# zacz08/ADM

Hardware: AMD Instinct MI355X
Metric: train images/sec (CIFAR-10 32x32 uncond DDM UNet, 1 optimizer step/iter) + 10-step sample images/sec (higher is better)
Workload: dtype f32; 1 GPU; BASELINE configs[1]: CIFAR-10 32x32 uncond two-decoder DhariwalUNet (216M params), bs=128/GPU fp32, ddm_const schedule, dropout 0.1, loss_simple (LPIPS term needs unfetchable VGG16 weights), clip 1.0 + AdamW + EMA(every 8); global_batch=128, image=3x32x32, parallelism=dp1, valid=True

## Files before the change

### adm_amd/csrc/conv_gemm_x6.hip

```cpp
#include "common.h"
#include "split_format.h"
#include <type_traits>

namespace {

struct G6P {
  const float* x; const unsigned short* w; const float* bias; const float* res; float* y;
  int M, N, K, ldx, ldy, ldr, wrows, tilesN, xbytes, wbytes, ybytes, rbytes;
  const float* amax_x; float wscale;
  float* amax_y;
};

typedef __attribute__((address_space(3))) void g6_lds_void;
constexpr int GM = 128, GN = 128, GCH = 2;
template <int FMT> struct G6Fmt {
  static constexpr int TERMS = split_terms(FMT);
  static constexpr int IMG = GCH * TERMS * 128 * 16;
  static constexpr int QW = 2 * TERMS;
};
constexpr int G_RA = 2, G_RB = 4, G_D = 4;

template <int FMT>
__global__ __launch_bounds__(512) void gemm_x6_kernel(G6P p) {
  constexpr int G_IMG = G6Fmt<FMT>::IMG, TERMS = G6Fmt<FMT>::TERMS, QW = G6Fmt<FMT>::QW;
  float sa = 1.f, inv_scale = 1.f;
  if (FMT) { sa = split_scale(adm_amax_read(p.amax_x)); inv_scale = 1.f / (sa * p.wscale); }
  extern __shared__ __attribute__((aligned(16))) unsigned short smg[];
  unsigned short* As = smg;
  unsigned short* Bs = smg + G_RA * G_IMG;
  const int tid = threadIdx.x, lane = tid & 63, hw_wid = tid >> 6;
  const bool producer = hw_wid >= 4;
  const int wid = hw_wid & 3;
  const int bid = adm_xcd_remap(blockIdx.x, gridDim.x);
  const int tilesM = gridDim.x / p.tilesN;
  const int tm = bid % tilesM, tn = bid / tilesM;
  const int m0 = tm * GM, n0 = tn * GN;
  const int S = p.K >> 5;
  constexpr unsigned OOB = 0x80000000u;

  if (producer) {
    const __amdgpu_buffer_rsrc_t rs_x = __builtin_amdgcn_make_buffer_rsrc(const_cast<float*>(p.x), 0, p.xbytes, 0x00020000);
    const int ptid = wid * 64 + lane;
    const int prow = ptid >> 3, quad = ptid & 7;
    unsigned voff[4];
#pragma unroll
    for (int j = 0; j < 4; ++j) {
      const int m = m0 + prow + 32 * j;
      voff[j] = (m < p.M) ? (unsigned)(((long)m * p.ldx + quad * 4) * 4) : OOB;
    }
    const int aq = quad & 3, ch = quad >> 2;
    unsigned short* la[4];
#pragma unroll
    for (int j = 0; j < 4; ++j) {
      const int row = prow + 32 * j;
      la[j] = As + (ch * TERMS * 128 + row) * 16 + ((((aq >> 1) ^ (row >> 3)) & 1) << 3) + (aq & 1) * 4;
    }
    f32x4 d[G_D][4];
    auto issue = [&](int set, int s) {
      const int soff = s << 7;
#pragma unroll
      for (int j = 0; j < 4; ++j)
        d[set][j] = __builtin_bit_cast(f32x4, __builtin_amdgcn_raw_buffer_load_b128(rs_x, (int)(s < S ? voff[j] : OOB), soff, 0));
    };
    auto store = [&](int set, int slot) {
#pragma unroll
      for (int j = 0; j < 4; ++j) {
        unsigned short* l = la[j] + slot * G_IMG;
        if (FMT) {
          u32x2 h0, h1;
          split2_quad(d[set][j], sa, h0, h1);
          *reinterpret_cast<u32x2*>(l) = h0;
          *reinterpret_cast<u32x2*>(l + 128 * 16) = h1;
          continue;
        }
        u32x2 t0, t1, t2;
        split3_quad(d[set][j], t0, t1, t2);
        *reinterpret_cast<u32x2*>(l) = t0;
        *reinterpret_cast<u32x2*>(l + 128 * 16) = t1;
        *reinterpret_cast<u32x2*>(l + 2 * 128 * 16) = t2;
      }
    };
#pragma unroll
    for (int k = 0; k < G_D; ++k) issue(k, k);
    __builtin_amdgcn_sched_barrier(0);
    for (int s0 = 0; s0 < S; s0 += G_D) {
#pragma unroll
      for (int k = 0; k < G_D; ++k) {
        if (s0 + k < S) {
          store(k, k & 1);
          __builtin_amdgcn_sched_barrier(0);
          issue(k, s0 + k + G_D);
          __builtin_amdgcn_sched_barrier(0);
          adm_lds_barrier();
        }
      }
    }
    return;
  }

  const __amdgpu_buffer_rsrc_t rs_w = __builtin_amdgcn_make_buffer_rsrc(const_cast<unsigned short*>(p.w), 0, p.wbytes, 0x00020000);
  const int wm = wid >> 1, wn = wid & 1;
  const int lr = lane & 31, lh = lane >> 5;
  unsigned b_voff[QW];
#pragma unroll
  for (int i = 0; i < QW; ++i) {
    const int q = wid * QW + i, img = q >> 2;
    const int row = (q & 3) * 32 + (lane >> 1);
    const int n = n0 + row;
    const int half = (lane ^ (row >> 3)) & 1;
    b_voff[i] = (n < p.wrows) ? (unsigned)((((long)img * p.wrows + n) * 16 + half * 8) * 2) : OOB;
  }
  int ld_s = 0, ld_slot = 0;
  auto issue_b = [&]() {
    const int kb = (ld_s * GCH * TERMS * p.wrows) << 5;
    unsigned short* dst = Bs + ld_slot * G_IMG + (wid * QW) * 512;
#pragma unroll
    for (int i = 0; i < QW; ++i)
      __builtin_amdgcn_raw_ptr_buffer_load_lds(rs_w, (g6_lds_void*)(dst + i * 512), 16, (int)b_voff[i], kb, 0, 0);
    ++ld_s;
    if (++ld_slot == G_RB) ld_slot = 0;
  };

  f32x16 acc[2][2], tot[2][2];
#pragma unroll
  for (int a = 0; a < 2; ++a)
#pragma unroll
    for (int b = 0; b < 2; ++b)
#pragma unroll
      for (int r = 0; r < 16; ++r) tot[a][b][r] = 0.f;
  const int fh = ((lh ^ (lr >> 3)) & 1) * 8;
  const int a_foff = (wm * 64 + lr) * 16 + fh;
  const int b_foff = (wn * 64 + lr) * 16 + fh;
  const f32x16 zero = {0.f, 0.f, 0.f, 0.f, 0.f, 0.f, 0.f, 0.f, 0.f, 0.f, 0.f, 0.f, 0.f, 0.f, 0.f, 0.f};

  issue_b();
  if (S > 1) issue_b();
  if (S > 2) issue_b();
  int slot_b = 0;
  for (int s = 0; s < S; ++s) {
    if (s + 2 < S) { if (FMT) asm volatile("s_waitcnt vmcnt(8) lgkmcnt(0)\n\ts_barrier" ::: "memory"); else asm volatile("s_waitcnt vmcnt(12) lgkmcnt(0)\n\ts_barrier" ::: "memory"); }
    else if (s + 1 < S) { if (FMT) asm volatile("s_waitcnt vmcnt(4) lgkmcnt(0)\n\ts_barrier" ::: "memory"); else asm volatile("s_waitcnt vmcnt(6) lgkmcnt(0)\n\ts_barrier" ::: "memory"); }
    else asm volatile("s_waitcnt vmcnt(0) lgkmcnt(0)\n\ts_barrier" ::: "memory");
    if (s + 3 < S) issue_b();
    const unsigned short* Ab = As + (s & 1) * G_IMG + a_foff;
    const unsigned short* Bb = Bs + slot_b * G_IMG + b_foff;
    if (++slot_b == G_RB) slot_b = 0;
    const bool first = (s & 1) == 0;
#pragma unroll
    for (int ch = 0; ch < GCH; ++ch) {
      bf16x8 a[2][TERMS], b[2][TERMS];
#pragma unroll
      for (int k = 0; k < TERMS; ++k)
#pragma unroll
        for (int blk = 0; blk < 2; ++blk) {
          a[blk][k] = __builtin_bit_cast(bf16x8, *reinterpret_cast<const u32x4*>(Ab + ((ch * TERMS + k) * 128 + blk * 32) * 16));
          b[blk][k] = __builtin_bit_cast(bf16x8, *reinterpret_cast<const u32x4*>(Bb + ((ch * TERMS + k) * 128 + blk * 32) * 16));
        }
#pragma unroll
      for (int mi = 0; mi < 2; ++mi)
#pragma unroll
        for (int ni = 0; ni < 2; ++ni) {
          f32x16 c;
          if (FMT) {
            const f16x8 a0 = __builtin_bit_cast(f16x8, a[mi][0]), a1 = __builtin_bit_cast(f16x8, a[mi][1]);
            const f16x8 b0 = __builtin_bit_cast(f16x8, b[ni][0]), b1 = __builtin_bit_cast(f16x8, b[ni][1]);
            c = __builtin_amdgcn_mfma_f32_32x32x16_f16(a0, b1, (first && ch == 0) ? zero : acc[mi][ni], 0, 0, 0);
            c = __builtin_amdgcn_mfma_f32_32x32x16_f16(a1, b0, c, 0, 0, 0);
            acc[mi][ni] = __builtin_amdgcn_mfma_f32_32x32x16_f16(a0, b0, c, 0, 0, 0);
            continue;
          }
          if (first && ch == 0) c = __builtin_amdgcn_mfma_f32_32x32x16_bf16(a[mi][0], b[ni][TERMS - 1], zero, 0, 0, 0);
          else c = __builtin_amdgcn_mfma_f32_32x32x16_bf16(a[mi][0], b[ni][TERMS - 1], acc[mi][ni], 0, 0, 0);
#ifndef G6_HALF
          c = __builtin_amdgcn_mfma_f32_32x32x16_bf16(a[mi][TERMS - 1], b[ni][0], c, 0, 0, 0);
          c = __builtin_amdgcn_mfma_f32_32x32x16_bf16(a[mi][1], b[ni][1], c, 0, 0, 0);
          c = __builtin_amdgcn_mfma_f32_32x32x16_bf16(a[mi][0], b[ni][1], c, 0, 0, 0);
#endif
          c = __builtin_amdgcn_mfma_f32_32x32x16_bf16(a[mi][1], b[ni][0], c, 0, 0, 0);
          acc[mi][ni] = __builtin_amdgcn_mfma_f32_32x32x16_bf16(a[mi][0], b[ni][0], c, 0, 0, 0);
        }
    }
    if (!first || s + 1 == S) {
#pragma unroll
      for (int mi = 0; mi < 2; ++mi)
#pragma unroll
        for (int ni = 0; ni < 2; ++ni) tot[mi][ni] += acc[mi][ni];
    }
  }

  const __amdgpu_buffer_rsrc_t rs_y = __builtin_amdgcn_make_buffer_rsrc(p.y, 0, p.ybytes, 0x00020000);
  const __amdgpu_buffer_rsrc_t rs_r = __builtin_amdgcn_make_buffer_rsrc(const_cast<float*>(p.res), 0, p.res ? p.rbytes : 0, 0x00020000);
  float am = 0.f;
  auto epilogue = [&](auto res_tag) {
    constexpr bool RES = decltype(res_tag)::value;
    float bv[2];
#pragma unroll
    for (int ni = 0; ni < 2; ++ni) {
      const int n = n0 + wn * 64 + ni * 32 + lr;
      bv[ni] = (p.bias && n < p.N) ? p.bias[n] : 0.f;
    }
    float v[2][2][16];
    unsigned n4[2], cmask[2], oy[2][16];
#pragma unroll
    for (int ni = 0; ni < 2; ++ni) {
      const int n = n0 + wn * 64 + ni * 32 + lr;
      n4[ni] = (unsigned)n * 4u;
      cmask[ni] = n < p.N ? 0u : OOB;
    }
    if (RES) {
      unsigned orr[2][16];
#pragma unroll
      for (int mi = 0; mi < 2; ++mi)
#pragma unroll
        for (int r = 0; r < 16; ++r) {
          const int m = m0 + wm * 64 + mi * 32 + 4 * lh + (r & 3) + 8 * (r >> 2);
          orr[mi][r] = m < p.M ? (unsigned)m * (unsigned)p.ldr * 4u : OOB;
        }
#pragma unroll
      for (int ni = 0; ni < 2; ++ni)
#pragma unroll
        for (int mi = 0; mi < 2; ++mi)
#pragma unroll
          for (int r = 0; r < 16; ++r)
            v[ni][mi][r] = __builtin_bit_cast(float, __builtin_amdgcn_raw_buffer_load_b32(rs_r, (int)max(orr[mi][r] + n4[ni], cmask[ni]), 0, 0));
      __builtin_amdgcn_sched_barrier(0);
    }
#pragma unroll
    for (int mi = 0; mi < 2; ++mi)
#pragma unroll
      for (int r = 0; r < 16; ++r) {
        const int m = m0 + wm * 64 + mi * 32 + 4 * lh + (r & 3) + 8 * (r >> 2);
        oy[mi][r] = m < p.M ? (unsigned)m * (unsigned)p.ldy * 4u : OOB;
      }
#pragma unroll
    for (int ni = 0; ni < 2; ++ni)
#pragma unroll
      for (int mi = 0; mi < 2; ++mi)
#pragma unroll
        for (int r = 0; r < 16; ++r) {
          v[ni][mi][r] = (FMT ? tot[mi][ni][r] * inv_scale : tot[mi][ni][r]) + bv[ni] + (RES ? v[ni][mi][r] : 0.f);
          am = fmaxf(am, (int)(oy[mi][r] | cmask[ni]) >= 0 ? fabsf(v[ni][mi][r]) : 0.f);
        }
    __builtin_amdgcn_sched_barrier(0);
#pragma unroll
    for (int ni = 0; ni < 2; ++ni)
#pragma unroll
      for (int mi = 0; mi < 2; ++mi)
#pragma unroll
        for (int r = 0; r < 16; ++r)
          __builtin_amdgcn_raw_buffer_store_b32(__builtin_bit_cast(unsigned, v[ni][mi][r]), rs_y, (int)max(oy[mi][r] + n4[ni], cmask[ni]), 0, 0);
  };
  if (p.res) epilogue(std::true_type{});
  else epilogue(std::false_type{});
  adm_amax_commit(am, p.amax_y);
}

__global__ void split3_rows_kernel(const float* __restrict__ src, unsigned short* __restrict__ dst, int rows, int cols, int ld) {
  const long total = (long)rows * cols;
  for (long i = blockIdx.x * (long)blockDim.x + threadIdx.x; i < total; i += (long)gridDim.x * blockDim.x) {
    const int n = (int)(i / cols), c = (int)(i - (long)n * cols);
    split3_store(src[(long)n * ld + c], dst + rows_image_offset(3, rows, n, c), split_term_stride(rows));
  }
}

__global__ void split2_rows_kernel(const float* __restrict__ src, unsigned short* __restrict__ dst, int rows, int cols, int ld, float scale,
                                   int* __restrict__ overflow) {
  const long total = (long)rows * cols;
  bool bad = false;
  for (long i = blockIdx.x * (long)blockDim.x + threadIdx.x; i < total; i += (long)gridDim.x * blockDim.x) {
    const int n = (int)(i / cols), c = (int)(i - (long)n * cols);
    const float a = src[(long)n * ld + c] * scale;
    bad |= split_f16_overflow(a);
    split2_store(a, dst + rows_image_offset(2, rows, n, c), split_term_stride(rows));
  }
  if (bad && overflow) *overflow = 1;
}

}

extern "C" int adm_split3_rows(const float* src, void* dst, int rows, int cols, int ld, hipStream_t stream) {
  if (!src || !dst || rows <= 0 || cols <= 0 || (cols & 15) || ld < cols) return ADM_EINVAL;
  const long total = (long)rows * cols;
  const int grid = (int)((total + 255) / 256 > 4096 ? 4096 : (total + 255) / 256);
  hipLaunchKernelGGL(split3_rows_kernel, dim3(grid), dim3(256), 0, stream, src, static_cast<unsigned short*>(dst), rows, cols, ld);
  ADM_CHECK_LAUNCH();
  return ADM_OK;
}

static int gemm_x6_launch(const float* x, const void* w6, const float* bias, const float* res, float* y, long M, int K, int ldx, int N,
                          int wrows, int ldy, int ldr, hipStream_t stream, const float* amax_x, float wscale, float* amax_y) {
  const bool h3 = amax_x != nullptr;
  if (!x || !w6 || !y || M <= 0 || K <= 0 || (K & 31) || (ldx & 3) || N <= 0 || wrows < N) return ADM_EINVAL;
  if (((uintptr_t)x | (uintptr_t)w6) & 15) return ADM_EINVAL;
  if (h3 && !(wscale > 0.f)) return ADM_EINVAL;
  G6P p;
  p.x = x; p.w = static_cast<const unsigned short*>(w6); p.bias = bias; p.res = res; p.y = y;
  p.amax_x = amax_x; p.wscale = wscale; p.amax_y = amax_y;
  const long xb = M * ldx * 4, wb = (h3 ? 2L : 3L) * wrows * K * 2, yb = M * ldy * 4, rb = res ? M * ldr * 4 : 0;
  if (M >= (1L << 30) || xb >= (1L << 31) || wb >= (1L << 31) || yb >= (1L << 31) || rb >= (1L << 31)) return ADM_EINVAL;
  p.M = (int)M; p.N = N; p.K = K; p.ldx = ldx; p.ldy = ldy; p.ldr = ldr; p.wrows = wrows;
  p.xbytes = (int)xb; p.wbytes = (int)wb; p.ybytes = (int)yb; p.rbytes = (int)rb;
  p.tilesN = adm_cdiv(N, GN);
  constexpr int smem0 = (G_RA + G_RB) * G6Fmt<0>::IMG * (int)sizeof(unsigned short), smem1 = (G_RA + G_RB) * G6Fmt<1>::IMG * (int)sizeof(unsigned short);
  static bool attr_set = false;
  if (!attr_set) {
    if (hipFuncSetAttribute(reinterpret_cast<const void*>(&gemm_x6_kernel<0>), hipFuncAttributeMaxDynamicSharedMemorySize, smem0) != hipSuccess ||
        hipFuncSetAttribute(reinterpret_cast<const void*>(&gemm_x6_kernel<1>), hipFuncAttributeMaxDynamicSharedMemorySize, smem1) != hipSuccess)
      return ADM_ELAUNCH;
    attr_set = true;
  }
  const long grid = (long)adm_cdiv(M, GM) * p.tilesN;
  if (h3) hipLaunchKernelGGL(gemm_x6_kernel<1>, dim3((unsigned)grid), dim3(512), smem1, stream, p);
  else hipLaunchKernelGGL(gemm_x6_kernel<0>, dim3((unsigned)grid), dim3(512), smem0, stream, p);
  ADM_CHECK_LAUNCH();
  return ADM_OK;
}

extern "C" int adm_gemm_x6(const float* x, const void* w6, const float* bias, const float* res, float* y, long M, int K, int ldx, int N,
                           int wrows, int ldy, int ldr, hipStream_t stream) {
  return gemm_x6_launch(x, w6, bias, res, y, M, K, ldx, N, wrows, ldy, ldr, stream, nullptr, 0.f, nullptr);
}
extern "C" int adm_gemm_x6_amax(const float* x, const void* w6, const float* bias, const float* res, float* y, long M, int K, int ldx, int N,
                                int wrows, int ldy, int ldr, float* amax_y, hipStream_t stream) {
  return gemm_x6_launch(x, w6, bias, res, y, M, K, ldx, N, wrows, ldy, ldr, stream, nullptr, 0.f, amax_y);
}
extern "C" int adm_gemm_x6_h3(const float* x, const void* wh, const float* bias, const float* res, float* y, long M, int K, int ldx, int N,
                              int wrows, int ldy, int ldr, const float* amax_x, float wscale, float* amax_y, hipStream_t stream) {
  if (!amax_x) return ADM_EINVAL;
  return gemm_x6_launch(x, wh, bias, res, y, M, K, ldx, N, wrows, ldy, ldr, stream, amax_x, wscale, amax_y);
}
extern "C" int adm_split2_rows_f16(const float* src, void* dst, int rows, int cols, int ld, float scale, int* overflow, hipStream_t stream) {
  if (!src || !dst || rows <= 0 || cols <= 0 || (cols & 15) || ld < cols || !(scale > 0.f)) return ADM_EINVAL;
  const long total = (long)rows * cols;
  const int grid = (int)((total + 255) / 256 > 4096 ? 4096 : (total + 255) / 256);
  hipLaunchKernelGGL(split2_rows_kernel, dim3(grid), dim3(256), 0, stream, src, static_cast<unsigned short*>(dst), rows, cols, ld, scale, overflow);
  ADM_CHECK_LAUNCH();
  return ADM_OK;
}
```

### adm_amd/hip.py

```python
from __future__ import annotations

import ctypes
import os
import subprocess
from ctypes import c_double, c_float, c_int, c_long, c_uint64, c_void_p

import torch

_HERE = os.path.dirname(os.path.abspath(__file__))
LIB_PATH = os.path.join(_HERE, "libadm_hip.so")
_lib = None

P, I, L, F, D, U = c_void_p, c_int, c_long, c_float, c_double, c_uint64
_SIGS = {
    "adm_version": [],
    "adm_conv_fwd": [P, P, P, P, P, I, I, I, I, I, I, I, I, I, I, I, I, P],
    "adm_conv_splitk": [I, I, I],
    "adm_conv_fwd_ws": [P, P, P, P, P, P, L, I, I, I, I, I, I, I, I, I, I, I, P],
    "adm_conv_fwd_strided": [P, P, P, P, P, I, I, I, I, I, I, I, I, I, I, I, I, I, I, P],
    "adm_conv_fwd_wino": [P, P, P, P, P, I, I, I, I, I, I, I, I, I, P],
    "adm_conv_fwd_wino_up": [P, P, P, P, P, I, I, I, I, I, I, I, I, I, P],
    "adm_pack_weight_wino": [P, P, P, I, I, I, I, P],
    "adm_pack_weight_wino2d": [P, P, P, I, I, I, I, P],
    "adm_conv_fwd_wino2d": [P, P, P, P, P, P, L, I, I, I, I, I, I, I, I, I, P],
    "adm_wino2d_splitk": [I, I, I, I, I],
    "adm_wino2d_variant": [I],
    "adm_wino2d_h3_wide": [I],
    "adm_wgrad_h3_blocks": [I],
    "adm_conv_fwd_wino2d_x6": [P, P, P, P, P, P, L, I, I, I, I, I, I, I, I, I, P],
    "adm_conv_fwd_wino2d_x6_up": [P, P, P, P, P, P, L, I, I, I, I, I, I, I, I, I, P],
    "adm_wino2d_x6_splitk": [I, I, I, I, I],
    "adm_split3_bf16": [P, P, I, I, P],
    "adm_split2_f16": [P, P, I, I, F, P, P],
    "adm_conv_fwd_wino2d_h3": [P, P, P, P, P, P, L, I, I, I, I, I, I, I, I, I, P, F, I, P],
    "adm_gemm_x6": [P, P, P, P, P, L, I, I, I, I, I, I, P],
    "adm_gemm_x6_amax": [P, P, P, P, P, L, I, I, I, I, I, I, P, P],
    "adm_gemm_x6_h3": [P, P, P, P, P, L, I, I, I, I, I, I, P, F, P, P],
    "adm_split2_rows_f16": [P, P, I, I, I, F, P, P],
    "adm_split3_rows": [P, P, I, I, I, P],
    "adm_conv_wgrad_x6": [P, P, P, P, I, I, I, I, I, I, I, I, P],
    "adm_conv_wgrad_x6_up": [P, P, P, P, I, I, I, I, I, I, I, I, P],
    "adm_conv_wgrad_x6_ws": [P, P, P, P, I, I, I, I, I, I, I, I, I, P],
    "adm_conv_wgrad_x6_plan": [I, I, I, I, I],
    "adm_gemm_wgrad_x6": [P, P, P, P, L, I, I, I, I, I, P],
    "adm_gemm_wgrad_x6_ws": [P, P, P, P, L, I, I, I, I, I, P],
    "adm_gemm_wgrad_x6_plan": [L, I, I],
    "adm_conv_wgrad_x6_h3": [P, P, P, P, I, I, I, I, I, I, I, I, I, I, P, P, P],
    "adm_gemm_wgrad_x6_h3": [P, P, P, P, L, I, I, I, I, I, I, P, P, P],
    "adm_conv_wgrad_x6_bf16a": [P, P, P, P, I, I, I, I, I, I, I, I, I, P],
    "adm_gemm_wgrad_x6_bf16a": [P, P, P, P, L, I, I, I, I, I, P],
    "adm_conv_wgrad": [P, P, P, I, I, I, I, I, I, I, I, I, I, P],
    "adm_conv_wgrad_wino": [P, P, P, P, I, I, I, I, I, I, I, I, P],
    "adm_conv_wgrad_wino_up": [P, P, P, P, I, I, I, I, I, I, I, I, P],
    "adm_conv_wgrad_bias": [P, P, P, P, I, I, I, I, I, I, I, I, I, I, P],
    "adm_conv_wgrad_wino2d": [P, P, P, P, I, I, I, I, I, I, I, I, P],
    "adm_unpack_wgrad_wino2d": [P, I, P, I, I, I, I, I, P, P, P],
    "adm_conv_wgrad_plan": [I, I, I, I, I, I, I, I],
    "adm_conv_wgrad_ws": [P, P, P, P, I, I, I, I, I, I, I, I, I, I, I, P],
    "adm_unpack_wgrad_splits": [P, I, P, I, I, I, I, I, I, I, P, P, P],
    "adm_conv_fwd_bf16": [P, P, P, P, P, I, I, I, I, I, I, I, I, I, I, I, I, P],
    "adm_conv_wgrad_bf16": [P, P, P, I, I, I, I, I, I, I, I, I, I, P],
    "adm_conv_fwd_bf16a": [P, P, P, P, P, I, I, I, I, I, I, I, I, I, I, I, I, P],
    "adm_conv_wgrad_bf16a": [P, P, P, I, I, I, I, I, I, I, I, I, I, P],
    "adm_gn_fwd_bf16out": [P, P, P, P, P, P, L, P, I, I, I, I, F, I, F, U, P],
    "adm_f32_to_bf16": [P, P, L, P],
    "adm_pack_weight": [P, P, P, I, I, I, I, I, I, P],
    "adm_pack_weight_table": [P, I, L, P],
    "adm_unpack_wgrad_table": [P, I, L, P],
    "adm_gn_bwd_param_table": [P, I, L, P],
    "adm_unpack_wgrad": [P, P, I, I, I, I, I, I, I, P],
    "adm_permute_vec": [P, P, I, I, I, I, P],
    "adm_colsum": [P, P, I, I, I, I, P],
    "adm_gn_splits": [I, I],
    "adm_gn_fused": [I],
    "adm_gn_plan": [I, I, I, P],
    "adm_gn_stats": [P, P, P, I, I, I, I, F, P],
    "adm_gn_apply": [P, P, P, P, P, L, P, I, I, I, I, I, F, U, P],
    "adm_gn_fwd": [P, P, P, P, P, P, L, P, I, I, I, I, F, I, F, U, P],
    "adm_gn_fwd_amax": [P, P, P, P, P, P, L, P, P, I, I, I, I, F, I, F, U, P],
    "adm_gn_bwd": [P, P, P, P, P, P, L, P, P, P, P, P, I, I, I, I, I, F, U, P],
    "adm_gn_bwd_add": [P, P, P, P, P, P, L, P, P, P, P, P, P, I, I, I, I, I, F, U, P],
    "adm_gn_bwd_add_amax": [P, P, P, P, P, P, L, P, P, P, P, P, P, P, I, I, I, I, I, F, U, P],
    "adm_gn_fwd_cat_amax": [P, I, P, I, F, P, P, P, P, P, P, P, L, P, P, I, I, I, F, I, F, U, P],
    "adm_gn_bwd_add_cat_amax": [P, P, P, P, P, P, L, P, P, I, P, I, F, P, P, P, P, P, I, I, I, I, F, U, P],
    "adm_softmax_rows": [P, L, I, L, F, P],
    "adm_posterior_sample": [P, I, P, P, I, L, I, F, P],
    "adm_attn_fwd": [P, P, P, I, I, I, P],
    "adm_attn_bwd": [P, P, P, P, P, P, I, I, I, P],
    "adm_attn_bwd_amax": [P, P, P, P, P, P, P, I, I, I, P],
    "adm_attn_fwd_h3": [P, P, P, P, I, I, I, P],
    "adm_attn_bwd_h3": [P, P, P, P, P, P, P, P, P, I, I, I, P],
    "adm_resample2x": [P, P, I, I, I, I, I, F, I, P],
    "adm_nchw_to_nhwc": [P, I, P, L, P, I, I, I, I, P],
    "adm_nchw_to_nhwc_amax": [P, I, P, L, P, P, I, I, I, I, P],
    "adm_precond_out": [P, I, P, I, P, P, L, P, I, I, I, P],
    "adm_precond_out_bwd": [P, P, L, P, I, I, I, I, P],
    "adm_precond_out_bwd_amax": [P, P, L, P, I, P, I, I, I, P],
    "adm_axpby_b": [P, I, P, P, P, L, P, I, L, P],
    "adm_pos_embedding": [P, P, I, I, P],
    "adm_silu_fwd": [P, P, L, P],
    "adm_silu_bwd": [P, P, P, L, P],
    "adm_add": [P, P, P, L, P],
    "adm_add3": [P, P, P, P, P, L, P],
    "adm_copy_channels": [P, I, I, P, I, I, L, I, F, I, P],
    "adm_concat2": [P, I, P, I, P, L, F, P, P],
    "adm_split2": [P, P, I, P, I, L, F, P],
    "adm_spatial_att_fwd": [P, I, P, P, P, P, I, I, I, P],
    "adm_spatial_att_bwd": [P, I, P, P, P, P, P, P, P, I, I, I, P],
    "adm_q_sample": [P, P, P, P, I, L, I, P],
    "adm_ddm_loss": [P, P, P, P, P, P, P, P, F, I, L, P],
    "adm_ddm_loss_latent": [P, P, P, P, P, P, P, P, P, P, P, F, I, L, I, I, P],
    "adm_ddm_loss_l1": [P, P, P, P, P, P, P, P, F, I, L, P],
    "adm_sampler_step": [P, P, P, D, D, I, I, D, I, L, P],
    "adm_sampler_step_stochastic": [P, P, P, P, P, P, I, I, D, I, I, L, P],
    "adm_q_sample_linear": [P, P, P, P, P, I, L, P],
    "adm_ddm_loss_linear": [P, P, P, P, P, P, P, P, P, P, P, P, I, L, I, P],
    "adm_sampler_step_linear": [P, P, P, P, P, P, F, I, I, L, P],
    "adm_nhwc_to_nchw": [P, I, P, I, I, I, P],
    "adm_nhwc_to_nchw_bwd_amax": [P, P, I, P, I, I, I, P],
    "adm_aug_workspace_floats": [I, I, I, I],
    "adm_augment_geometric": [P, P, P, P, P, P, I, I, I, I, P],
# ... 18 lines not shown
    "adm_spatial_att_big_bwd": [P, I, P, P, P, P, P, P, P, P, I, I, I, P],
    "adm_mha_fwd": [P, P, P, P, P, I, I, I, I, I, I, I, I, I, F, P],
    "adm_mha_bwd": [P, P, P, P, P, P, P, P, P, P, I, I, I, I, I, I, I, I, I, I, I, I, F, P],
    "adm_linattn_ws_floats": [I, I],
    "adm_linattn_fwd": [P, P, P, P, P, I, I, P],
    "adm_linattn_bwd": [P, P, P, P, P, P, P, P, I, I, P],
    "adm_sumsq_blocks": [L],
    "adm_sumsq": [P, P, P, L, P],
    "adm_adamw_step": [P, P, P, P, P, P, L, F, D, D, F, F, F, I, D, F, P],
    "adm_lpips_input": [P, P, P, P, P, P, P, I, I, I, P],
    "adm_lpips_input_bwd": [P, P, P, P, P, I, I, I, P],
    "adm_lpips_input_c1": [P, P, P, P, P, P, P, I, I, I, P],
    "adm_lpips_input_c1_bwd": [P, P, P, P, P, I, I, I, P],
    "adm_maxpool2x2_fwd": [P, P, I, I, I, I, P],
    "adm_maxpool2x2_bwd": [P, P, P, I, I, I, I, P],
    "adm_lpips_head_blocks": [I],
    "adm_lpips_head_fwd": [P, P, P, P, P, I, I, I, I, P],
    "adm_lpips_head_bwd": [P, P, P, P, P, I, I, I, P],
    "adm_ae_blocks": [L],
    "adm_posterior_kl_fwd": [P, I, P, P, I, P, P, I, L, I, P],
    "adm_posterior_kl_bwd": [P, I, P, P, I, P, P, I, L, I, P],
    "adm_ae_nll_fwd": [P, P, P, P, P, P, I, L, F, P],
    "adm_ae_nll_bwd": [P, P, P, F, P, L, P],
    "adm_logit_terms_fwd": [P, I, P, P, L, P],
    "adm_logit_terms_bwd": [P, I, I, P, F, P, L, P],
    "adm_leaky_relu_fwd": [P, P, L, F, P],
    "adm_leaky_relu_bwd": [P, P, P, L, F, P],
    "adm_softmax_rows_bwd": [P, P, L, I, L, F, P],
    "adm_transpose2d": [P, P, I, I, P],
    "adm_adaptive_weight": [P, L, P, L, P, F, P, P],
    "adm_axpy_dev": [P, P, P, F, P, L, P],
    "adm_swin_attn_fwd": [P, P, P, P, I, I, I, I, I, I, I, I, P],
    "adm_ln_affine_fwd": [P, P, P, P, L, I, F, P],
    "adm_swin_merge_ln_fwd": [P, P, P, P, I, I, I, I, F, P],
    "adm_swin_attn_bwd_ws_floats": [I, I, I, I],
    "adm_swin_attn_bwd": [P, P, P, P, P, P, P, P, I, I, I, I, I, I, I, I, I, I, P],
    "adm_ln_bwd_ws_floats": [L, I],
    "adm_ln_affine_bwd": [P, P, P, P, P, P, P, L, I, F, I, P],
    "adm_swin_merge_ln_bwd": [P, P, P, P, P, P, P, I, I, I, I, F, I, P],
    "adm_rowscale_add": [P, P, P, P, I, L, P],
    "adm_patch_embed_ln_fwd": [P, P, P, P, P, P, I, I, I, I, F, P],
    "adm_patch_embed_ln_bwd_ws_floats": [I, I, I, I],
    "adm_patch_embed_ln_bwd": [P, P, P, P, P, P, P, P, P, P, I, I, I, I, F, I, P],
    "adm_sr_tile": [I],
    "adm_sr_batch": [P, L, P, P, I, P, P, P, P, P, P, I, P, P, I, P, P, P, I, I, I, I, I, P],
    "adm_inpaint_masks": [P, P, P, P, P, P, P, P, P, I, I, P],
    "adm_inpaint_batch": [P, L, P, P, I, P, P, P, P, P, P, P, P, P, P, I, I, P],
    "adm_inpaint_compose": [P, P, P, P, I, I, L, P],
    "adm_pair_resize_lds": [I, I, I, I, I, I],
    "adm_pair_resize_batch": [P, L, P, P, P, L, P, P, I, P, L, P, I, P, I, I, I, I, P, P, P, P, P, P, I, I, I, P],
    "adm_image_resize_batch": [P, L, P, P, I, I, P, L, P, I, P, I, I, I, I, P, P, P, P, I, I, I, P],
    "adm_conv_rect_relu_fwd": [P, P, P, P, I, I, I, I, I, I, I, I, I, I, I, I, I, I, I, P],
    "adm_pool3x3_fwd": [P, P, I, I, I, I, I, I, I, I, P],
    "adm_global_avgpool_fwd": [P, P, I, I, I, I, I, P],
    "adm_tf1_resize_norm_u8": [P, P, I, I, I, P],
    "adm_feat_stats_accum": [P, I, I, P, P, P, I, P],
}
EXPORTS = tuple(_SIGS)


def build(verbose: bool = False) -> str:
    r = subprocess.run(["make", "-C", os.path.join(_HERE, "csrc"), "-j8"], capture_output=True, text=True)
    if verbose or r.returncode != 0:
        print(r.stdout[-4000:], r.stderr[-8000:])
    if r.returncode != 0 or not os.path.exists(LIB_PATH):
        raise RuntimeError("building libadm_hip.so failed")
    return LIB_PATH


def lib() -> ctypes.CDLL:
    global _lib
    if _lib is None:
        if not os.path.exists(LIB_PATH):
            raise RuntimeError(f"{LIB_PATH} is missing: run `python -c 'import __graft_entry__ as g; g.build()'` "
                               "(there is no non-HIP fallback for the adm_amd hot path)")
        _lib = ctypes.CDLL(LIB_PATH)
        for name, args in _SIGS.items():
            fn = getattr(_lib, name)
            fn.argtypes = args
            fn.restype = c_long if name in ("adm_aug_workspace_floats", "adm_linattn_ws_floats", "adm_swin_attn_bwd_ws_floats",
                                        "adm_ln_bwd_ws_floats", "adm_pair_resize_lds", "adm_patch_embed_ln_bwd_ws_floats") else c_int
        if os.environ.get("ADM_H3_WIDE") is not None:
            _lib.adm_wino2d_h3_wide(int(os.environ["ADM_H3_WIDE"]))
        if os.environ.get("ADM_WGRAD_H3_BLOCKS") is not None:
            _lib.adm_wgrad_h3_blocks(int(os.environ["ADM_WGRAD_H3_BLOCKS"]))
    return _lib


def stream() -> c_void_p:
    return c_void_p(torch.cuda.current_stream().cuda_stream)


def ptr(t) -> c_void_p:
    return None if t is None else c_void_p(t.data_ptr())


NO_STREAM = ("adm_version", "adm_conv_splitk", "adm_gn_splits", "adm_aug_workspace_floats", "adm_conv_wgrad_plan",
             "adm_sumsq_blocks", "adm_lnc_blocks", "adm_bn_blocks", "adm_linattn_ws_floats", "adm_wino2d_splitk", "adm_wino2d_x6_splitk", "adm_wino2d_variant", "adm_wino2d_h3_wide", "adm_wgrad_h3_blocks", "adm_gn_fused", "adm_gn_plan", "adm_conv_wgrad_x6_plan", "adm_gemm_wgrad_x6_plan", "adm_lpips_head_blocks", "adm_ae_blocks", "adm_swin_attn_bwd_ws_floats", "adm_ln_bwd_ws_floats", "adm_sr_tile", "adm_pair_resize_lds", "adm_patch_embed_ln_bwd_ws_floats")


def call(name: str, *args):
    rc = getattr(lib(), name)(*args, stream())
    if rc != 0:
        raise RuntimeError(f"{name} failed with code {rc} (-22 = unsupported shape/alignment, -5 = launch failure)")


def require_cuda(t: torch.Tensor, what: str = "tensor"):
    if not t.is_cuda:
        raise RuntimeError(f"adm_amd: {what} is on {t.device}; the HIP hot path needs a GPU tensor "
                           "(no CPU fallback exists by design)")
```

### include/adm_hip.h

```cpp
#ifndef ADM_HIP_H
#define ADM_HIP_H
#include <stdint.h>
typedef struct ihipStream_t* hipStream_t;

#ifdef __cplusplus
#define ADM_AMAX_SLOTS 64
#define ADM_AMAX_STRIDE 32
#define ADM_AMAX_FLOATS (ADM_AMAX_SLOTS * ADM_AMAX_STRIDE)

extern "C" {
#endif

int adm_version(void);


int adm_conv_fwd(const float* x, const float* wp, const float* bias, const float* res, float* y,
                 int B, int H, int W, int Cin, int ldx, int N, int wrows, int ldy, int ldr,
                 int ks, int up, int tile, hipStream_t stream);

int adm_conv_fwd_strided(const float* x, const float* wp, const float* bias, const float* res, float* y,
                         int B, int Hin, int Win, int Hout, int Wout, int Cin, int ldx, int N, int wrows,
                         int ldy, int ldr, int ks, int stride, int pad_lo, hipStream_t stream);

int adm_conv_fwd_wino(const float* x, const float* wq, const float* bias, const float* res, float* y, int B, int H, int W,
                      int Cin, int ldx, int N, int wrows, int ldy, int ldr, hipStream_t stream);
int adm_conv_fwd_wino_up(const float* x, const float* wq, const float* bias, const float* res, float* y, int B, int H, int W,
                         int Cin, int ldx, int N, int wrows, int ldy, int ldr, hipStream_t stream);
int adm_pack_weight_wino(const float* w, float* wf, float* wb, int Co, int Ci, int Co_pad, int Ci_pad, hipStream_t stream);

int adm_conv_splitk(int M, int N, int K);
int adm_conv_fwd_ws(const float* x, const float* wp, const float* bias, const float* res, float* y, float* ws,
                    long ws_floats, int B, int H, int W, int Cin, int ldx, int N, int wrows, int ldy, int ldr, int ks,
                    int up, hipStream_t stream);

int adm_conv_wgrad(const float* x, const float* dy, float* dwp, int B, int H, int W, int Cin, int ldx,
                   int Cout, int lddy, int ks, int up, int splits, hipStream_t stream);

int adm_conv_wgrad_bias(const float* x, const float* dy, float* dwp, float* dbias, int B, int H, int W, int Cin, int ldx,
                        int Cout, int lddy, int ks, int up, int splits, hipStream_t stream);

int adm_conv_wgrad_wino(const float* x, const float* dy, float* dwp, float* dbias, int B, int H, int W, int Cin, int ldx,
                        int Cout, int lddy, int splits, hipStream_t stream);

int adm_conv_wgrad_wino_up(const float* x, const float* dy, float* dwp, float* dbias, int B, int H, int W, int Cin, int ldx,
                           int Cout, int lddy, int splits, hipStream_t stream);

int adm_pack_weight_wino2d(const float* w, float* wf, float* wb, int Co, int Ci, int Co_pad, int Ci_pad, hipStream_t stream);
int adm_conv_fwd_wino2d(const float* x, const float* wq, const float* bias, const float* res, float* y, float* ws, long ws_floats,
                        int B, int H, int W, int Cin, int ldx, int N, int wrows, int ldy, int ldr, hipStream_t stream);
int adm_conv_fwd_wino2d_x6(const float* x, const void* wq6, const float* bias, const float* res, float* y, float* ws,
                           long ws_floats, int B, int H, int W, int Cin, int ldx, int N, int wrows, int ldy, int ldr,
                           hipStream_t stream);
int adm_conv_fwd_wino2d_x6_up(const float* x, const void* wq6, const float* bias, const float* res, float* y, float* ws,
                              long ws_floats, int B, int H, int W, int Cin, int ldx, int N, int wrows, int ldy, int ldr,
                              hipStream_t stream);
int adm_wino2d_x6_splitk(int B, int H, int W, int Cin, int N);
int adm_split2_f16(const float* src, void* dst, int rows, int cols, float scale, int* overflow, hipStream_t stream);
int adm_conv_fwd_wino2d_h3(const float* x, const void* wqh, const float* bias, const float* res, float* y, float* ws,
                           long ws_floats, int B, int H, int W, int Cin, int ldx, int N, int wrows, int ldy, int ldr,
                           const float* amax_x, float wscale, int up, hipStream_t stream);
int adm_split3_bf16(const float* src, void* dst, int rows, int cols, hipStream_t stream);
int adm_gemm_x6(const float* x, const void* w6, const float* bias, const float* res, float* y, long M, int K, int ldx, int N, int wrows,
                int ldy, int ldr, hipStream_t stream);
int adm_split3_rows(const float* src, void* dst, int rows, int cols, int ld, hipStream_t stream);
int adm_gemm_x6_amax(const float* x, const void* w6, const float* bias, const float* res, float* y, long M, int K, int ldx, int N,
                     int wrows, int ldy, int ldr, float* amax_y, hipStream_t stream);
int adm_gemm_x6_h3(const float* x, const void* wh, const float* bias, const float* res, float* y, long M, int K, int ldx, int N, int wrows,
                   int ldy, int ldr, const float* amax_x, float wscale, float* amax_y, hipStream_t stream);
int adm_split2_rows_f16(const float* src, void* dst, int rows, int cols, int ld, float scale, int* overflow, hipStream_t stream);
int adm_conv_wgrad_x6(const float* x, const float* dy, float* dwp2, float* dbias, int B, int H, int W, int Cin, int ldx, int Cout,
                      int lddy, int splits, hipStream_t stream);
int adm_conv_wgrad_x6_up(const float* x, const float* dy, float* dwp2, float* dbias, int B, int H, int W, int Cin, int ldx, int Cout,
                         int lddy, int splits, hipStream_t stream);
int adm_conv_wgrad_x6_ws(const float* x, const float* dy, float* ws, float* bws, int B, int H, int W, int Cin, int ldx, int Cout,
                         int lddy, int splits, int up, hipStream_t stream);
int adm_conv_wgrad_x6_plan(int B, int H, int W, int Cin, int Cout);
int adm_gemm_wgrad_x6(const float* x, const float* dy, float* dwp, float* dbias, long P, int Cin, int ldx, int Cout, int lddy,
                      int splits, hipStream_t stream);
int adm_gemm_wgrad_x6_ws(const float* x, const float* dy, float* ws, float* bws, long P, int Cin, int ldx, int Cout, int lddy,
                         int splits, hipStream_t stream);
int adm_gemm_wgrad_x6_plan(long P, int Cin, int Cout);
int adm_conv_wgrad_x6_bf16a(const void* x16, const float* dy, float* dwp2, float* dbias, int B, int H, int W, int Cin, int ldx,
                            int Cout, int lddy, int splits, int up, hipStream_t stream);
int adm_gemm_wgrad_x6_bf16a(const void* x16, const float* dy, float* dwp, float* dbias, long P, int Cin, int ldx, int Cout, int lddy,
                            int splits, hipStream_t stream);
int adm_conv_wgrad_x6_h3(const float* x, const float* dy, float* dwp2, float* dbias, int B, int H, int W, int Cin, int ldx, int Cout,
                         int lddy, int splits, int up, int det, const float* amax_x, const float* amax_dy, hipStream_t stream);
int adm_gemm_wgrad_x6_h3(const float* x, const float* dy, float* dwp, float* dbias, long P, int Cin, int ldx, int Cout, int lddy,
                         int splits, int det, const float* amax_x, const float* amax_dy, hipStream_t stream);
int adm_wino2d_variant(int ws);
int adm_wino2d_h3_wide(int v);
int adm_wgrad_h3_blocks(int v);
int adm_wino2d_splitk(int B, int H, int W, int Cin, int N);

int adm_conv_wgrad_wino2d(const float* x, const float* dy, float* dwp2, float* dbias, int B, int H, int W, int Cin, int ldx,
                          int Cout, int lddy, int splits, hipStream_t stream);
int adm_unpack_wgrad_wino2d(const float* wx, int splits, float* dw, int Co, int Ci, int Co_pad, int Ci_pad, int accumulate,
                            const float* bws, float* dbias, hipStream_t stream);

int adm_conv_wgrad_plan(int B, int H, int W, int Cin, int Cout, int ks, int up, int wino);
int adm_conv_wgrad_ws(const float* x, const float* dy, float* ws, float* bws, int B, int H, int W, int Cin, int ldx, int Cout,
                      int lddy, int ks, int up, int splits, int wino, hipStream_t stream);

int adm_conv_fwd_bf16(const float* x, const unsigned short* wp16, const float* bias, const float* res, float* y,
                      int B, int H, int W, int Cin, int ldx, int N, int wrows, int ldy, int ldr, int ks, int up,
                      int tile, hipStream_t stream);
int adm_conv_wgrad_bf16(const float* x, const float* dy, float* dwp, int B, int H, int W, int Cin, int ldx, int Cout,
                        int lddy, int ks, int up, int splits, hipStream_t stream);
int adm_conv_fwd_bf16a(const void* x16, const unsigned short* wp16, const float* bias, const float* res, float* y, int B, int H, int W,
                       int Cin, int ldx, int N, int wrows, int ldy, int ldr, int ks, int up, int tile, hipStream_t stream);
int adm_conv_wgrad_bf16a(const void* x16, const float* dy, float* dwp, int B, int H, int W, int Cin, int ldx, int Cout, int lddy, int ks,
                         int up, int splits, hipStream_t stream);
int adm_gn_fwd_bf16out(const float* x, float* stats, double* ws, const float* gamma, const float* beta, const float* ss,
                       long ss_bstride, void* y16, int B, int HW, int C, int G, float eps, int silu, float drop_p, uint64_t seed,
                       hipStream_t stream);
int adm_f32_to_bf16(const float* src, unsigned short* dst, long n, hipStream_t stream);

int adm_pack_weight(const float* w, float* wp_fwd, float* wp_bwd, int Co, int Ci, int ks, int Co_pad, int Ci_pad,
                    int qkv, hipStream_t stream);
int adm_pack_weight_table(const long* table, int n_entries, long total_tiles, hipStream_t stream);
int adm_unpack_wgrad(const float* dwp, float* dw, int Co, int Ci, int ks, int Co_pad, int Ci_pad, int qkv,
                     int accumulate, hipStream_t stream);
int adm_unpack_wgrad_splits(const float* ws, int splits, float* dw, int Co, int Ci, int ks, int Co_pad, int Ci_pad, int qkv,
                            int accumulate, const float* bws, float* dbias, hipStream_t stream);
int adm_unpack_wgrad_table(const long* table, int rows, long total_blocks, hipStream_t stream);
int adm_permute_vec(const float* in, float* out, int n, int n_pad, int qkv, int inverse, hipStream_t stream);
int adm_colsum(const float* a, float* out, int M, int N, int ld, int accumulate, hipStream_t stream);


int adm_gn_fused(int on);
int adm_gn_splits(int HW, int C);
int adm_gn_plan(int HW, int C, int G, int* out);
int adm_gn_stats(const float* x, float* stats, double* ws, int B, int HW, int C, int G, float eps, hipStream_t stream);
int adm_gn_apply(const float* x, const float* stats, const float* gamma, const float* beta, const float* ss,
                 long ss_bstride, float* y, int B, int HW, int C, int G, int silu, float drop_p, uint64_t seed,
                 hipStream_t stream);
int adm_gn_fwd(const float* x, float* stats, double* ws, const float* gamma, const float* beta, const float* ss,
               long ss_bstride, float* y, int B, int HW, int C, int G, float eps, int silu, float drop_p, uint64_t seed,
               hipStream_t stream);
int adm_gn_fwd_amax(const float* x, float* stats, double* ws, const float* gamma, const float* beta, const float* ss,
                    long ss_bstride, float* y, float* amax, int B, int HW, int C, int G, float eps, int silu, float drop_p,
                    uint64_t seed, hipStream_t stream);
int adm_gn_bwd(const float* x, const float* dy, const float* stats, const float* gamma, const float* beta,
               const float* ss, long ss_bstride, float* dx, float* dss, float* dgamma, float* dbeta, float* red,
               int B, int HW, int C, int G, int silu, float drop_p, uint64_t seed, hipStream_t stream);

int adm_gn_bwd_param_table(const long* table, int rows, long total_blocks, hipStream_t stream);

int adm_gn_bwd_add(const float* x, const float* dy, const float* stats, const float* gamma, const float* beta,
                   const float* ss, long ss_bstride, const float* addend, float* dx, float* dss, float* dgamma, float* dbeta,
                   float* red, int B, int HW, int C, int G, int silu, float drop_p, uint64_t seed, hipStream_t stream);
int adm_gn_bwd_add_amax(const float* x, const float* dy, const float* stats, const float* gamma, const float* beta,
// ... 277 lines not shown
```

Before: 1267 images/s.

## Add wider N-tile variants to split-f16 GEMM with cost-based selection

Templates the x6 GEMM kernel on an N-block count, so the fp16-split path can use 128, 192 or 256-column tiles with 4, 6 or 8 consumer waves plus 4 producer waves. A heuristic picks the tile width per shape from a wave-count cost model, with an env override and a plan query exposed to Python. Wider tiles reuse each A tile across more columns and cut redundant A loads and workgroups. The cost is more LDS and threads per block, which may lower occupancy.

```diff
diff --git a/adm_amd/csrc/conv_gemm_x6.hip b/adm_amd/csrc/conv_gemm_x6.hip
--- a/adm_amd/csrc/conv_gemm_x6.hip
+++ b/adm_amd/csrc/conv_gemm_x6.hip
@@ -12,29 +12,37 @@
 };
 
 typedef __attribute__((address_space(3))) void g6_lds_void;
-constexpr int GM = 128, GN = 128, GCH = 2;
-template <int FMT> struct G6Fmt {
+constexpr int GM = 128, GCH = 2;
+template <int FMT, int NB = 2> struct G6Fmt {
   static constexpr int TERMS = split_terms(FMT);
-  static constexpr int IMG = GCH * TERMS * 128 * 16;
-  static constexpr int QW = 2 * TERMS;
+  static constexpr int NT = 64 * NB;
+  static constexpr int CONS = 2 * NB;
+  static constexpr int THREADS = (CONS + 4) * 64;
+  static constexpr int A_IMG = GCH * TERMS * GM * 16;
+  static constexpr int B_IMG = GCH * TERMS * NT * 16;
+  static constexpr int RG = NT / 32;
+  static constexpr int QW = GCH * TERMS * RG / CONS;
+  static constexpr int SMEM = (2 * A_IMG + 4 * B_IMG) * (int)sizeof(unsigned short);
 };
 constexpr int G_RA = 2, G_RB = 4, G_D = 4;
 
-template <int FMT>
-__global__ __launch_bounds__(512) void gemm_x6_kernel(G6P p) {
-  constexpr int G_IMG = G6Fmt<FMT>::IMG, TERMS = G6Fmt<FMT>::TERMS, QW = G6Fmt<FMT>::QW;
+template <int FMT, int NB>
+__global__ __launch_bounds__((2 * NB + 4) * 64) void gemm_x6_kernel(G6P p) {
+  using F = G6Fmt<FMT, NB>;
+  constexpr int A_IMG = F::A_IMG, B_IMG = F::B_IMG, TERMS = F::TERMS, QW = F::QW, NT = F::NT, CONS = F::CONS, RG = F::RG;
+  static_assert(QW == 2 * TERMS, "the vmcnt immediates of the stage loop count 2 TERMS weight instructions per wave and stage");
   float sa = 1.f, inv_scale = 1.f;
   if (FMT) { sa = split_scale(adm_amax_read(p.amax_x)); inv_scale = 1.f / (sa * p.wscale); }
   extern __shared__ __attribute__((aligned(16))) unsigned short smg[];
   unsigned short* As = smg;
-  unsigned short* Bs = smg + G_RA * G_IMG;
+  unsigned short* Bs = smg + G_RA * A_IMG;
   const int tid = threadIdx.x, lane = tid & 63, hw_wid = tid >> 6;
-  const bool producer = hw_wid >= 4;
-  const int wid = hw_wid & 3;
+  const bool producer = hw_wid >= CONS;
+  const int wid = producer ? hw_wid - CONS : hw_wid;
   const int bid = adm_xcd_remap(blockIdx.x, gridDim.x);
   const int tilesM = gridDim.x / p.tilesN;
   const int tm = bid % tilesM, tn = bid / tilesM;
-  const int m0 = tm * GM, n0 = tn * GN;
+  const int m0 = tm * GM, n0 = tn * NT;
   const int S = p.K >> 5;
   constexpr unsigned OOB = 0x80000000u;
 
@@ -65,7 +73,7 @@
     auto store = [&](int set, int slot) {
 #pragma unroll
       for (int j = 0; j < 4; ++j) {
-        unsigned short* l = la[j] + slot * G_IMG;
+        unsigned short* l = la[j] + slot * A_IMG;
         if (FMT) {
           u32x2 h0, h1;
           split2_quad(d[set][j], sa, h0, h1);
@@ -99,13 +107,13 @@
   }
 
   const __amdgpu_buffer_rsrc_t rs_w = __builtin_amdgcn_make_buffer_rsrc(const_cast<unsigned short*>(p.w), 0, p.wbytes, 0x00020000);
-  const int wm = wid >> 1, wn = wid & 1;
+  const int wm = wid / NB, wn = wid % NB;
   const int lr = lane & 31, lh = lane >> 5;
   unsigned b_voff[QW];
 #pragma unroll
   for (int i = 0; i < QW; ++i) {
-    const int q = wid * QW + i, img = q >> 2;
-    const int row = (q & 3) * 32 + (lane >> 1);
+    const int q = wid * QW + i, img = q / RG;
+    const int row = (q % RG) * 32 + (lane >> 1);
     const int n = n0 + row;
     const int half = (lane ^ (row >> 3)) & 1;
     b_voff[i] = (n < p.wrows) ? (unsigned)((((long)img * p.wrows + n) * 16 + half * 8) * 2) : OOB;
@@ -113,7 +121,7 @@
   int ld_s = 0, ld_slot = 0;
   auto issue_b = [&]() {
     const int kb = (ld_s * GCH * TERMS * p.wrows) << 5;
-    unsigned short* dst = Bs + ld_slot * G_IMG + (wid * QW) * 512;
+    unsigned short* dst = Bs + ld_slot * B_IMG + (wid * QW) * 512;
 #pragma unroll
     for (int i = 0; i < QW; ++i)
       __builtin_amdgcn_raw_ptr_buffer_load_lds(rs_w, (g6_lds_void*)(dst + i * 512), 16, (int)b_voff[i], kb, 0, 0);
@@ -142,8 +150,8 @@
     else if (s + 1 < S) { if (FMT) asm volatile("s_waitcnt vmcnt(4) lgkmcnt(0)\n\ts_barrier" ::: "memory"); else asm volatile("s_waitcnt vmcnt(6) lgkmcnt(0)\n\ts_barrier" ::: "memory"); }
     else asm volatile("s_waitcnt vmcnt(0) lgkmcnt(0)\n\ts_barrier" ::: "memory");
     if (s + 3 < S) issue_b();
-    const unsigned short* Ab = As + (s & 1) * G_IMG + a_foff;
-    const unsigned short* Bb = Bs + slot_b * G_IMG + b_foff;
+    const unsigned short* Ab = As + (s & 1) * A_IMG + a_foff;
+    const unsigned short* Bb = Bs + slot_b * B_IMG + b_foff;
     if (++slot_b == G_RB) slot_b = 0;
     const bool first = (s & 1) == 0;
 #pragma unroll
@@ -154,7 +162,7 @@
 #pragma unroll
         for (int blk = 0; blk < 2; ++blk) {
           a[blk][k] = __builtin_bit_cast(bf16x8, *reinterpret_cast<const u32x4*>(Ab + ((ch * TERMS + k) * 128 + blk * 32) * 16));
-          b[blk][k] = __builtin_bit_cast(bf16x8, *reinterpret_cast<const u32x4*>(Bb + ((ch * TERMS + k) * 128 + blk * 32) * 16));
+          b[blk][k] = __builtin_bit_cast(bf16x8, *reinterpret_cast<const u32x4*>(Bb + ((ch * TERMS + k) * NT + blk * 32) * 16));
         }
 #pragma unroll
       for (int mi = 0; mi < 2; ++mi)
@@ -287,6 +295,41 @@
   return ADM_OK;
 }
 
+static int g_gemm_h3_form = -1;
+extern "C" int adm_gemm_h3_form(int v) { const int old = g_gemm_h3_form; g_gemm_h3_form = v; return old; }
+
+static constexpr long GEMM_X6_COST[3] = {32, 45, 48};
+static int gemm_x6_form(long M, int N, bool h3) {
+  if (!h3) return 2;
+  if (g_gemm_h3_form >= 2 && g_gemm_h3_form <= 4) return g_gemm_h3_form;
+  if (N > 128 && N <= 192) return 3;
+  const long tilesM = adm_cdiv(M, GM);
+  int form = 2;
+  long best = -1;
+  for (int nb = 2; nb <= 4; ++nb) {
+    const long t = (tilesM * adm_cdiv(N, 64 * nb) + 255) / 256 * GEMM_X6_COST[nb - 2];
+    if (best < 0 || t < best) { best = t; form = nb; }
+  }
+  return form;
+}
+
+extern "C" int adm_gemm_x6_plan(long M, int N, int K, int h3, int* out) {
+  if (!out || M <= 0 || N <= 0 || K <= 0 || (K & 31) || M >= (1L << 30)) return ADM_EINVAL;
+  const int nb = gemm_x6_form(M, N, h3 != 0);
+  const long wgs = (long)adm_cdiv(M, GM) * adm_cdiv(N, 64 * nb);
+  out[0] = nb;
+  out[1] = (2 * nb + 4) * 64;
+  out[2] = !h3 ? G6Fmt<0>::SMEM : nb == 2 ? G6Fmt<1, 2>::SMEM : nb == 3 ? G6Fmt<1, 3>::SMEM : G6Fmt<1, 4>::SMEM;
+  out[3] = (int)wgs;
+  out[4] = (int)((wgs + 255) / 256);
+  return ADM_OK;
+}
+
+template <int FMT, int NB> static void gemm_x6_go(dim3 grid, hipStream_t stream, const G6P& p) {
+  using F = G6Fmt<FMT, NB>;
+  hipLaunchKernelGGL((gemm_x6_kernel<FMT, NB>), grid, dim3(F::THREADS), F::SMEM, stream, p);
+}
+
 static int gemm_x6_launch(const float* x, const void* w6, const float* bias, const float* res, float* y, long M, int K, int ldx, int N,
                           int wrows, int ldy, int ldr, hipStream_t stream, const float* amax_x, float wscale, float* amax_y) {
   const bool h3 = amax_x != nullptr;
@@ -300,18 +343,22 @@
   if (M >= (1L << 30) || xb >= (1L << 31) || wb >= (1L << 31) || yb >= (1L << 31) || rb >= (1L << 31)) return ADM_EINVAL;
   p.M = (int)M; p.N = N; p.K = K; p.ldx = ldx; p.ldy = ldy; p.ldr = ldr; p.wrows = wrows;
   p.xbytes = (int)xb; p.wbytes = (int)wb; p.ybytes = (int)yb; p.rbytes = (int)rb;
-  p.tilesN = adm_cdiv(N, GN);
-  constexpr int smem0 = (G_RA + G_RB) * G6Fmt<0>::IMG * (int)sizeof(unsigned short), smem1 = (G_RA + G_RB) * G6Fmt<1>::IMG * (int)sizeof(unsigned short);
   static bool attr_set = false;
   if (!attr_set) {
-    if (hipFuncSetAttribute(reinterpret_cast<const void*>(&gemm_x6_kernel<0>), hipFuncAttributeMaxDynamicSharedMemorySize, smem0) != hipSuccess ||
-        hipFuncSetAttribute(reinterpret_cast<const void*>(&gemm_x6_kernel<1>), hipFuncAttributeMaxDynamicSharedMemorySize, smem1) != hipSuccess)
+    if (hipFuncSetAttribute(reinterpret_cast<const void*>(&gemm_x6_kernel<0, 2>), hipFuncAttributeMaxDynamicSharedMemorySize, G6Fmt<0>::SMEM) != hipSuccess ||
+        hipFuncSetAttribute(reinterpret_cast<const void*>(&gemm_x6_kernel<1, 2>), hipFuncAttributeMaxDynamicSharedMemorySize, G6Fmt<1, 2>::SMEM) != hipSuccess ||
+        hipFuncSetAttribute(reinterpret_cast<const void*>(&gemm_x6_kernel<1, 3>), hipFuncAttributeMaxDynamicSharedMemorySize, G6Fmt<1, 3>::SMEM) != hipSuccess ||
+        hipFuncSetAttribute(reinterpret_cast<const void*>(&gemm_x6_kernel<1, 4>), hipFuncAttributeMaxDynamicSharedMemorySize, G6Fmt<1, 4>::SMEM) != hipSuccess)
       return ADM_ELAUNCH;
     attr_set = true;
   }
-  const long grid = (long)adm_cdiv(M, GM) * p.tilesN;
-  if (h3) hipLaunchKernelGGL(gemm_x6_kernel<1>, dim3((unsigned)grid), dim3(512), smem1, stream, p);
-  else hipLaunchKernelGGL(gemm_x6_kernel<0>, dim3((unsigned)grid), dim3(512), smem0, stream, p);
+  const int nb = gemm_x6_form(M, N, h3);
+  p.tilesN = adm_cdiv(N, 64 * nb);
+  const dim3 grid((unsigned)((long)adm_cdiv(M, GM) * p.tilesN));
+  if (!h3) gemm_x6_go<0, 2>(grid, stream, p);
+  else if (nb == 2) gemm_x6_go<1, 2>(grid, stream, p);
+  else if (nb == 3) gemm_x6_go<1, 3>(grid, stream, p);
+  else gemm_x6_go<1, 4>(grid, stream, p);
   ADM_CHECK_LAUNCH();
   return ADM_OK;
 }
diff --git a/adm_amd/hip.py b/adm_amd/hip.py
--- a/adm_amd/hip.py
+++ b/adm_amd/hip.py
@@ -37,6 +37,8 @@
     "adm_gemm_x6_amax": [P, P, P, P, P, L, I, I, I, I, I, I, P, P],
     "adm_gemm_x6_h3": [P, P, P, P, P, L, I, I, I, I, I, I, P, F, P, P],
     "adm_split2_rows_f16": [P, P, I, I, I, F, P, P],
+    "adm_gemm_h3_form": [I],
+    "adm_gemm_x6_plan": [L, I, I, I, P],
     "adm_split3_rows": [P, P, I, I, I, P],
     "adm_conv_wgrad_x6": [P, P, P, P, I, I, I, I, I, I, I, I, P],
     "adm_conv_wgrad_x6_up": [P, P, P, P, I, I, I, I, I, I, I, I, P],
@@ -221,6 +223,8 @@
                                         "adm_ln_bwd_ws_floats", "adm_pair_resize_lds", "adm_patch_embed_ln_bwd_ws_floats") else c_int
         if os.environ.get("ADM_H3_WIDE") is not None:
             _lib.adm_wino2d_h3_wide(int(os.environ["ADM_H3_WIDE"]))
+        if os.environ.get("ADM_GEMM_H3_FORM") is not None:
+            _lib.adm_gemm_h3_form(int(os.environ["ADM_GEMM_H3_FORM"]))
         if os.environ.get("ADM_WGRAD_H3_BLOCKS") is not None:
             _lib.adm_wgrad_h3_blocks(int(os.environ["ADM_WGRAD_H3_BLOCKS"]))
     return _lib
@@ -235,7 +239,7 @@
 
 
 NO_STREAM = ("adm_version", "adm_conv_splitk", "adm_gn_splits", "adm_aug_workspace_floats", "adm_conv_wgrad_plan",
-             "adm_sumsq_blocks", "adm_lnc_blocks", "adm_bn_blocks", "adm_linattn_ws_floats", "adm_wino2d_splitk", "adm_wino2d_x6_splitk", "adm_wino2d_variant", "adm_wino2d_h3_wide", "adm_wgrad_h3_blocks", "adm_gn_fused", "adm_gn_plan", "adm_conv_wgrad_x6_plan", "adm_gemm_wgrad_x6_plan", "adm_lpips_head_blocks", "adm_ae_blocks", "adm_swin_attn_bwd_ws_floats", "adm_ln_bwd_ws_floats", "adm_sr_tile", "adm_pair_resize_lds", "adm_patch_embed_ln_bwd_ws_floats")
+             "adm_sumsq_blocks", "adm_lnc_blocks", "adm_bn_blocks", "adm_linattn_ws_floats", "adm_wino2d_splitk", "adm_wino2d_x6_splitk", "adm_wino2d_variant", "adm_wino2d_h3_wide", "adm_wgrad_h3_blocks", "adm_gemm_h3_form", "adm_gemm_x6_plan", "adm_gn_fused", "adm_gn_plan", "adm_conv_wgrad_x6_plan", "adm_gemm_wgrad_x6_plan", "adm_lpips_head_blocks", "adm_ae_blocks", "adm_swin_attn_bwd_ws_floats", "adm_ln_bwd_ws_floats", "adm_sr_tile", "adm_pair_resize_lds", "adm_patch_embed_ln_bwd_ws_floats")
 
 
 def call(name: str, *args):
diff --git a/include/adm_hip.h b/include/adm_hip.h
--- a/include/adm_hip.h
+++ b/include/adm_hip.h
@@ -68,6 +68,8 @@
 int adm_gemm_x6_h3(const float* x, const void* wh, const float* bias, const float* res, float* y, long M, int K, int ldx, int N, int wrows,
                    int ldy, int ldr, const float* amax_x, float wscale, float* amax_y, hipStream_t stream);
 int adm_split2_rows_f16(const float* src, void* dst, int rows, int cols, int ld, float scale, int* overflow, hipStream_t stream);
+int adm_gemm_h3_form(int v);
+int adm_gemm_x6_plan(long M, int N, int K, int h3, int* out);
 int adm_conv_wgrad_x6(const float* x, const float* dy, float* dwp2, float* dbias, int B, int H, int W, int Cin, int ldx, int Cout,
                       int lddy, int splits, hipStream_t stream);
 int adm_conv_wgrad_x6_up(const float* x, const float* dy, float* dwp2, float* dbias, int B, int H, int W, int Cin, int ldx, int Cout,
```

Result: no change. 1277 images/s, median of 6 (+0.8%).
